# tprelle/janusgraph

Measured on AMD Instinct MI355X. Metric: GTEPS for PageRank iter + BFS, RMAT-24/26, 1/2/4/8 GPUs; % of HBM peak, higher is better.
Workload: dtype f64

## Files before the change

janusgraph_amd/csrc/jg_cc.hip:

```cpp
#include <climits>
#include <cstdio>
#include <cstdlib>

#include "jg_frontier.h"
#include "jg_pull.h"

namespace jg {

namespace {

constexpr int kCcMaxIterations = 100;

struct CcOp {
    using T = int32_t;
    const int32_t* __restrict__ msg;
    int32_t* __restrict__ msg_out;
    int32_t* __restrict__ label;
    int32_t* __restrict__ changed;
    VecPos pos;
    __device__ __forceinline__ int32_t identity() const { return INT_MAX; }
    __device__ __forceinline__ int32_t combine(int32_t a, int32_t b) const { return a < b ? a : b; }
    __device__ __forceinline__ int32_t gather(int32_t c) const { return msg[c]; }
    __device__ __forceinline__ const int32_t* vec() const { return msg; }
    __device__ __forceinline__ int32_t shfl_xor(int32_t v, int o) const { return __shfl_xor(v, o, kWave); }
    __device__ __forceinline__ int32_t shfl_up(int32_t v, int d) const { return __shfl_up(v, d, kWave); }
    __device__ __forceinline__ bool active(int64_t) const { return true; }
    __device__ __forceinline__ void finalize(int64_t row, int32_t m) const {
        if (m < label[row]) {
            label[row] = m;
            msg_out[pos(row)] = m;
            *changed = 1;
        } else {
            msg_out[pos(row)] = INT_MAX;
        }
    }
};

__device__ __forceinline__ int digits_of(uint64_t x) {
    int d = 1;
    while (d < 20 && x >= 10ull) { x /= 10ull; ++d; }
    return d;
}

__global__ void lex_digits_kernel(const int64_t* __restrict__ vid, int64_t n, uint64_t* __restrict__ keys,
                                  uint32_t* __restrict__ vals) {
    for (int64_t i = (int64_t)blockIdx.x * blockDim.x + threadIdx.x; i < n; i += (int64_t)gridDim.x * blockDim.x) {
        keys[i] = (uint64_t)digits_of((uint64_t)vid[i]);
        vals[i] = (uint32_t)i;
    }
}

__global__ void lex_padded_kernel(const int64_t* __restrict__ vid, const uint32_t* __restrict__ vals, int64_t n,
                                  uint64_t* __restrict__ keys) {
    for (int64_t i = (int64_t)blockIdx.x * blockDim.x + threadIdx.x; i < n; i += (int64_t)gridDim.x * blockDim.x) {
        uint64_t x = (uint64_t)vid[vals[i]];
        for (int d = digits_of(x); d < 19; ++d) x *= 10ull;
        keys[i] = x;
    }
}

__global__ void lex_rank_scatter_kernel(const uint32_t* __restrict__ vals, int64_t n, int32_t* __restrict__ rank_of) {
    for (int64_t r = (int64_t)blockIdx.x * blockDim.x + threadIdx.x; r < n; r += (int64_t)gridDim.x * blockDim.x)
        rank_of[vals[r]] = (int32_t)r;
}

__global__ void iota_i64_kernel(int64_t* __restrict__ p, int64_t n) {
    for (int64_t i = (int64_t)blockIdx.x * blockDim.x + threadIdx.x; i < n; i += (int64_t)gridDim.x * blockDim.x) p[i] = i;
}

__global__ void vid_of_rank_kernel(const uint32_t* __restrict__ vals, const int64_t* __restrict__ vid, int64_t n,
                                   int64_t* __restrict__ vor) {
    for (int64_t r = (int64_t)blockIdx.x * blockDim.x + threadIdx.x; r < n; r += (int64_t)gridDim.x * blockDim.x)
        vor[r] = vid[vals[r]];
}

__global__ void gather_i32_kernel(const int32_t* __restrict__ src, const int32_t* __restrict__ idx, int64_t n,
                                  int32_t* __restrict__ out) {
    for (int64_t i = (int64_t)blockIdx.x * blockDim.x + threadIdx.x; i < n; i += (int64_t)gridDim.x * blockDim.x)
// ... 1566 lines not shown
```

janusgraph_amd/csrc/jg_combine.hip:

```cpp
#include <climits>
#include <vector>

#include "jg_internal.h"
#include "jg_prim.h"
#include "jg_pull.h"

namespace jg {

namespace {

template <int OP>
struct Combine {
    __device__ static __forceinline__ int64_t identity() {
        return OP == JG_COMBINE_SUM ? 0 : OP == JG_COMBINE_MIN ? LLONG_MAX : LLONG_MIN;
    }
    __device__ static __forceinline__ int64_t apply(int64_t a, int64_t b) {
        if (OP == JG_COMBINE_SUM) return (int64_t)((uint64_t)a + (uint64_t)b);
        if (OP == JG_COMBINE_MIN) return b < a ? b : a;
        return b > a ? b : a;
    }
};

template <int OP>
__device__ __forceinline__ int64_t finish(int64_t acc, int wrap32) {
    return (OP == JG_COMBINE_SUM && wrap32) ? (int64_t)(int32_t)(uint32_t)acc : acc;
}

template <int OP>
struct CombOp {
    using T = long long;
    const long long* __restrict__ x;
    long long* __restrict__ x_out;
    VecPos pos;
    int wrap32;
    __device__ __forceinline__ long long identity() const { return Combine<OP>::identity(); }
    __device__ __forceinline__ long long combine(long long a, long long b) const { return Combine<OP>::apply(a, b); }
    __device__ __forceinline__ long long gather(int32_t c) const { return x[c]; }
    __device__ __forceinline__ const long long* vec() const { return x; }
    __device__ __forceinline__ long long shfl_xor(long long v, int o) const { return __shfl_xor(v, o, kWave); }
    __device__ __forceinline__ long long shfl_up(long long v, int d) const { return __shfl_up(v, d, kWave); }
    __device__ __forceinline__ bool active(int64_t) const { return true; }
    __device__ __forceinline__ void finalize(int64_t row, long long acc) const {
        x_out[pos(row)] = finish<OP>(acc, wrap32);
    }
};

__global__ void has_entries_kernel(const int64_t* __restrict__ row_ptr, int64_t rows, uint8_t* __restrict__ f) {
    for (int64_t r = (int64_t)blockIdx.x * blockDim.x + threadIdx.x; r < rows; r += (int64_t)gridDim.x * blockDim.x)
        f[r] = row_ptr[r + 1] > row_ptr[r];
}

template <int OP>
void launch_step(const Csr& c, const PullPlan& plan, long long* hub_partial, long long* split_partial,
                 const int64_t* x_in, int64_t* x_out, VecPos pos, int wrap32, hipStream_t s) {
    const CombOp<OP> op{reinterpret_cast<const long long*>(x_in), reinterpret_cast<long long*>(x_out), pos, wrap32};
    launch_pull(c, plan, op, hub_partial, s, nullptr, nullptr, split_partial);
}

}

void combine_run(Graph& g, int direction, int combiner, int wrap32, const int64_t* init, int steps, int64_t* out,
                 uint8_t* received_out) {
    if (direction < JG_DIR_OUT || direction > JG_DIR_BOTH) fail(JG_ERR_ARG, "direction must be JG_DIR_OUT/IN/BOTH");
    if (combiner < JG_COMBINE_SUM || combiner > JG_COMBINE_MAX) fail(JG_ERR_ARG, "unknown combiner");
    if (steps < 0) fail(JG_ERR_ARG, "negative step count");
    const uint32_t adj = direction == JG_DIR_OUT ? JG_ADJ_OUT : direction == JG_DIR_IN ? JG_ADJ_IN : JG_ADJ_BOTH;
    if (!(g.flags & adj))
        fail(JG_ERR_UNSUPPORTED, std::string("graph was built without the ") +
                                     (direction == JG_DIR_OUT ? "OUT" : direction == JG_DIR_IN ? "IN" : "BOTH") +
                                     " adjacency");
    const size_t ns = g.shards.size();
    struct St {
        DevBuf<int64_t> x[2];
        DevBuf<uint8_t> recv;
        DevBuf<long long> hub_partial, split_partial;
        int64_t len = 0;
        VecPos pos;
    };
    std::vector<St> st(ns);
    for (size_t i = 0; i < ns; ++i) {
        Shard& sh = *g.shards[i];
        DeviceGuard dg(sh);
        hipStream_t s = sh.stream;
        St& t = st[i];
        const Csr& c = adj == JG_ADJ_OUT ? sh.out : adj == JG_ADJ_IN ? sh.in : sh.both;
        if (adj == JG_ADJ_OUT) {
            t.len = g.padded_len();
            t.pos.base = (int64_t)sh.index * g.S;
            if (!sh.plan_out_built) {
                build_pull_plan(sh, sh.out, sh.plan_out, g.padded_len(), g.padded_len(), 8);
                sh.plan_out_built = true;
            }
        } else {
// ... 105 lines not shown
```

janusgraph_amd/csrc/jg_pagerank.hip:

```cpp
#include <cstdlib>

#include "jg_pull.h"
#include "jg_scatter.h"

namespace jg {

namespace {

struct PrOp {
    using T = double;
    const double* __restrict__ x;
    double* __restrict__ contrib_out;
    double* __restrict__ rank;
    const int32_t* __restrict__ outdeg;
    VecPos pos;
    double damping, teleport;
    bool write_rank;
    __device__ __forceinline__ double identity() const { return 0.0; }
    __device__ __forceinline__ double combine(double a, double b) const { return __dadd_rn(a, b); }
    __device__ __forceinline__ double gather(int32_t c) const { return x[c]; }
    __device__ __forceinline__ const double* vec() const { return x; }
    __device__ __forceinline__ double shfl_xor(double v, int o) const { return __shfl_xor(v, o, kWave); }
    __device__ __forceinline__ double shfl_up(double v, int d) const { return __shfl_up(v, d, kWave); }
    __device__ __forceinline__ bool active(int64_t) const { return true; }
    __device__ __forceinline__ void finalize(int64_t row, double s) const {
        const double r = __dadd_rn(__dmul_rn(damping, s), teleport);
        if (write_rank) rank[row] = r;
        contrib_out[pos(row)] = r / (double)outdeg[row];
    }
};

__global__ void pr_init_kernel(const int32_t* __restrict__ outdeg, int64_t rows, VecPos pos, double initial,
                               double* __restrict__ contrib, double* __restrict__ rank) {
    for (int64_t l = (int64_t)blockIdx.x * blockDim.x + threadIdx.x; l < rows; l += (int64_t)gridDim.x * blockDim.x) {
        rank[l] = initial;
        contrib[pos(l)] = initial / (double)outdeg[l];
    }
}

void exchange_contrib(Graph& g, int which) {
    std::vector<void*> bufs;
    for (auto& sp : g.shards) bufs.push_back(sp->pr_contrib[which].peer());
    exchange_vec(g, JG_ADJ_IN, bufs, sizeof(double), ncclFloat64);
}

}

void pagerank_begin(Graph& g, double damping, int64_t vertex_count) {
    if (!(g.flags & JG_ADJ_IN)) fail(JG_ERR_UNSUPPORTED, "PageRank needs a graph built with JG_ADJ_IN");
    if (vertex_count == 0) fail(JG_ERR_ARG, "vertexCount must be non-zero");
    for (auto& sp : g.shards) {
        Shard& sh = *sp;
        DeviceGuard dg(sh);
        const int64_t len = g.vec_len(sh, JG_ADJ_IN);
        for (int k = 0; k < 2; ++k) {
            if (sh.pr_contrib[k].size() != (size_t)len) sh.pr_contrib[k].alloc(len);
            JG_HIP(hipMemsetAsync(sh.pr_contrib[k].get(), 0, sh.pr_contrib[k].bytes(), sh.stream));
        }
        if (sh.pr_rank.size() != (size_t)std::max<int64_t>(sh.rows, 1)) {
            const char* f = std::getenv("JG_VDEV_FAULT");
            if (f && *f && *f != '0' && sh.index > 0) {
                DeviceGuard d0(*g.shards[0]);
                sh.pr_rank.alloc(std::max<int64_t>(sh.rows, 1));
            } else {
                sh.pr_rank.alloc(std::max<int64_t>(sh.rows, 1));
            }
        }
        if (sh.pr_hub_partial.size() != (size_t)std::max<int64_t>(sh.plan_in.num_chunks, 1))
            sh.pr_hub_partial.alloc(std::max<int64_t>(sh.plan_in.num_chunks, 1));
        if (sh.pr_split_partial.size() != (size_t)sh.plan_in.split_partial_len()) {
            sh.pr_split_partial.alloc(sh.plan_in.split_partial_len());
        }
        const double initial = 1.0 / (double)vertex_count;
        if (sh.rows > 0) {
            pr_init_kernel<<<grid_for(sh.rows), kBlock, 0, sh.stream>>>(sh.out_degree.get(), sh.rows,
                                                                        g.vec_pos(sh, JG_ADJ_IN), initial,
// ... 65 lines not shown
```

janusgraph_amd/csrc/jg_pull.h:

```cpp
#pragma once

#include "jg_internal.h"
#include "jg_prim.h"

namespace jg {

struct PullArgs {
    const int64_t* __restrict__ row_ptr;
    const int32_t* __restrict__ col;
    const int64_t* __restrict__ chunk_row;
    const int64_t* __restrict__ chunk_begin;
    const int64_t* __restrict__ chunk_end;
    const int64_t* __restrict__ hub_chunk_ptr;
    int64_t num_chunks;
    int64_t num_hub_rows;
    int64_t class_row_begin[kNumClasses];
    int64_t class_row_end[kNumClasses];
    int64_t class_block_begin[kNumClasses + 1];
    int64_t block_offset;
    int64_t skip_rows;
    int runs;
    int64_t run_begin[kRunMax + 1];
    int64_t run_ptr[kRunMax + 1];
};

inline PullArgs make_pull_args(const Csr& csr, const PullPlan& p, bool light = false) {
    PullArgs a;
    a.row_ptr = csr.row_ptr.get();
    a.col = csr.col.get();
    a.chunk_row = p.chunk_row.get();
    a.chunk_begin = p.chunk_begin.get();
    a.chunk_end = p.chunk_end.get();
    a.hub_chunk_ptr = p.hub_chunk_ptr.get();
    a.num_chunks = p.num_chunks;
    a.num_hub_rows = p.num_hub_rows;
    for (int c = 0; c < kNumClasses; ++c) {
        a.class_row_begin[c] = light ? p.light_row_begin[c] : p.class_row_begin[c];
        a.class_row_end[c] = light ? p.light_row_end[c] : p.class_row_end[c];
    }
    for (int c = 0; c <= kNumClasses; ++c) a.class_block_begin[c] = light ? p.light_block_begin[c] : p.class_block_begin[c];
    a.block_offset = 0;
    a.skip_rows = light ? p.split_rows : 0;
    a.runs = p.runs;
    for (int d = 0; d <= kRunMax; ++d) {
        a.run_begin[d] = p.run_begin[d];
        a.run_ptr[d] = p.run_ptr[d];
    }
    return a;
}

template <class Op>
struct GlobalGather {
    const Op& op;
// ... 146 lines not shown
            T t = red[0];
#pragma unroll
            for (int w = 1; w < kBlock / kWave; ++w) t = op.combine(t, red[w]);
            hub_partial[b] = t;
        }
        return;
    }
    pull_block_rows<Op, U>(a, op, GlobalGather<Op>{op}, b, (int)threadIdx.x);
}

template <class Op, int U>
__global__ __launch_bounds__(kBlock) void pull_kernel(PullArgs a, Op op, typename Op::T* __restrict__ hub_partial) {
    pull_block<Op, U>(a, op, hub_partial, (int64_t)blockIdx.x + a.block_offset);
}

template <class Op>
__global__ void pull_hub_finalize_kernel(PullArgs a, Op op, const typename Op::T* __restrict__ hub_partial) {
    using T = typename Op::T;
    for (int64_t h = (int64_t)blockIdx.x * blockDim.x + threadIdx.x; h < a.num_hub_rows;
         h += (int64_t)gridDim.x * blockDim.x) {
        const int64_t c0 = a.hub_chunk_ptr[h], c1 = a.hub_chunk_ptr[h + 1];
        if (a.chunk_row[c0] < a.skip_rows) continue;
        T acc = op.identity();
        for (int64_t k = c0; k < c1; ++k) acc = op.combine(acc, hub_partial[k]);
        op.finalize(a.chunk_row[c0], acc);
    }
}

constexpr int kMergeThreads = 1024;
constexpr int kMergeWaves = kMergeThreads / kWave;
constexpr int kMergeEpl = kMergeTask / kWave;
constexpr int kMergeLdsBytes = 160 * 1024;

struct MergeArgs {
    const uint4* __restrict__ pack_a;
    const uint32_t* __restrict__ pack_b;
    const uint8_t* __restrict__ heads;
    const int32_t* __restrict__ meta;
    const int64_t* __restrict__ sub_begin;
    const int64_t* __restrict__ sub_end;
    const int64_t* __restrict__ sub_base;
    int64_t tasks;
    int bits;
    int stage;
    const uint32_t* __restrict__ live;
};

struct HotSegs {
    int32_t hs = 0;
    int tbits = 31;
    int nseg = 1;
};

template <class Op>
struct SliceGather {
    using T = typename Op::T;
    const Op& op;
    lds_ptr<const T> lds;
    uint32_t hg;
    int sb;
    int bits;
    uint32_t hmask, h;
    uint32_t idcell;
    __device__ __forceinline__ bool is_hot(uint32_t loc) const { return ((loc >> 4) & ((1u << sb) - 1u)) < hg; }
    __device__ __forceinline__ T hot(uint32_t loc, bool valid) const {
        const uint32_t g = loc >> 4, j = g & ((1u << sb) - 1u), seg = g >> sb;
        return lds[valid && j < hg ? (((seg * hg + j) << 4) | (loc & 15u)) : idcell];
    }
    __device__ __forceinline__ int32_t col(uint32_t loc) const {
        const uint32_t x = (loc >> 4) << bits;
        const uint32_t hx = (x ^ (x >> 8) ^ (x >> 16) ^ (x >> 24)) & hmask;
        return (int32_t)(((x | (h ^ hx)) << 4) | (loc & 15u));
    }
    __device__ __forceinline__ T cold(uint32_t loc, bool valid, bool lds_on) const {
        T v = op.identity();
        if (valid && !(lds_on && is_hot(loc))) v = op.gather(col(loc));
        return v;
    }
};

template <int W>
__device__ __forceinline__ uint32_t unpack_entry(const uint32_t (&d)[W / 4], int u) {
    const int o = W * u, i = o >> 5, sh = o & 31;
    uint32_t v = d[i] >> sh;
    if (sh + W > 32) v |= d[i + 1] << (32 - sh);
    if constexpr (W < 32) v &= (1u << W) - 1u;
    return v;
}

template <class Op, bool LDS, int PW>
__global__ __launch_bounds__(kMergeThreads) void pull_merge_kernel(MergeArgs a, Op op, typename Op::T* __restrict__ partial,
                                                                   typename Op::T* __restrict__ carry, HotSegs hs,
                                                                   int temporal) {
    using T = typename Op::T;
    extern __shared__ __align__(16) unsigned char merge_lds[];
    const int S = 1 << a.bits;
    const int xs = S < kXcds ? S : kXcds;
    const int rep = kXcds / xs;
    const int per = S / xs;
    const int w = (int)(blockIdx.x >> 3), W = (int)(gridDim.x >> 3);
    const int xcd = (int)(blockIdx.x & (kXcds - 1));
    const int wave = threadIdx.x / kWave, lane = threadIdx.x % kWave;
    lds_ptr<T> hotv = (lds_ptr<T>)merge_lds;
    const int gshift = 4 + a.bits;
    const int hg = hs.hs >> gshift;
    const int nl = hs.nseg * hg;
    lds_ptr<T> stg = hotv + (nl * 16 + 1) + wave * a.stage;
    lds_ptr<uint32_t> tctr = (lds_ptr<uint32_t>)(hotv + (nl * 16 + 1) + kMergeWaves * a.stage);
    const int rounds = temporal ? per : 1;
    const uint32_t hmask = (1u << a.bits) - 1u;
    auto image_line = [&](int seg, int j, int hh) {
        const int64_t grp = ((int64_t)seg << (hs.tbits - gshift)) + j;
        return (grp << a.bits) + (int64_t)(hh ^ (sub_hash(grp << gshift) & hmask));
    };
    for (int rd = 0; rd < rounds; ++rd) {
    const int h = (xcd % xs) | ((temporal ? rd : w % per) << 3);
    const int64_t g = (int64_t)(temporal ? w : w / per) * rep + xcd / xs;
    const int64_t G = (int64_t)(temporal ? W : W / per) * rep;
    if constexpr (LDS) {
        if (rd > 0) __syncthreads();
        constexpr int kStage = 8;
        constexpr int kUnit = 16 / (int)sizeof(T);
        static_assert(16 % sizeof(T) == 0 && kUnit <= 16, "16-byte staging units");
        const unsigned char* src = reinterpret_cast<const unsigned char*>(op.vec());
        const int units = nl * 16 / kUnit;
        using u4 = uint32_t __attribute__((ext_vector_type(4)));
        lds_ptr<u4> hv4 = (lds_ptr<u4>)merge_lds;
        for (int q0 = 0; q0 < units; q0 += kStage * kMergeThreads) {
            u4 buf[kStage];
#pragma unroll
            for (int u = 0; u < kStage; ++u) {
                const int q = q0 + u * kMergeThreads + (int)threadIdx.x;
                const int i = q * kUnit, sg = i >> 4;
                int seg = 0, j = sg;
                if (hs.nseg > 1) {
                    seg = sg / hg;
                    j = sg - seg * hg;
                }
                buf[u] = u4{0, 0, 0, 0};
                if (q < units)
                    buf[u] = *reinterpret_cast<const u4*>(src + (image_line(seg, j, h) * 16 + (i & 15)) * (int64_t)sizeof(T));
            }
#pragma unroll
            for (int u = 0; u < kStage; ++u) {
                const int q = q0 + u * kMergeThreads + (int)threadIdx.x;
                if (q < units) hv4[q] = buf[u];
            }
        }
        if (threadIdx.x == 0) {
            hotv[nl * 16] = op.identity();
            *tctr = 0u;
        }
        __syncthreads();
    }
    const SliceGather<Op> lg{op,       hotv, (uint32_t)hg, hs.tbits - gshift, a.bits, (1u << a.bits) - 1u, (uint32_t)h,
                             (uint32_t)nl * 16u};
    const int64_t base = a.sub_base[h];
    const int64_t ntask = a.sub_base[h + 1] - base;
    const int64_t hbegin = a.sub_begin[h], hend = a.sub_end[h];
    constexpr bool dyn = LDS;
    const int64_t grot = (g + rd) % G;
    auto task_of = [&](int64_t j) { return j * G + grot; };
    auto grab = [&]() -> int64_t {
        uint32_t j = 0;
        if (lane == 0) j = __hip_atomic_fetch_add(tctr, 1u, __ATOMIC_RELAXED, __HIP_MEMORY_SCOPE_WORKGROUP);
        return task_of((int64_t)__builtin_amdgcn_readfirstlane(j));
    };
    int64_t jstat = wave;
    auto advance = [&]() -> int64_t {
        if (dyn) return grab();
        jstat += kMergeWaves;
        return task_of(jstat);
    };
    auto dead = [&](int64_t kk) -> bool {
        if (a.live == nullptr || kk >= ntask) return false;
        const uint64_t tt = (uint64_t)(base + kk);
        const uint32_t wd = __builtin_amdgcn_readfirstlane(a.live[tt >> 5]);
        return ((wd >> (tt & 31)) & 1u) == 0;
    };
    int64_t k = dyn ? grab() : task_of(jstat);
    while (dead(k)) k = advance();
    if (k >= ntask) continue;
    static_assert(kMergeEpl == 8, "a lane chunk is 8 entries");
    constexpr int DB = PW / 4 - 4;
    auto chunk = [&](int64_t kk) { return (hbegin >> 3) + kk * kWave + lane; };
    auto meta_idx = [&](int64_t kk) { return 2 * (base + kk) + (lane & 1); };
    auto head_idx = [&](int64_t kk) { return (base + kk) * kWave + lane; };
    auto ld = [](const auto* p) { return *p; };
    using v4u = uint32_t __attribute__((ext_vector_type(4)));
    using v2u = uint32_t __attribute__((ext_vector_type(2)));
    auto load_chunk = [&](int64_t kk, uint32_t (&d)[PW / 4]) {
        const int64_t x = chunk(kk);
        const v4u va = ld(reinterpret_cast<const v4u*>(a.pack_a) + x);
        d[0] = va.x, d[1] = va.y, d[2] = va.z, d[3] = va.w;
        if constexpr (DB == 1) {
            d[4] = ld(a.pack_b + x);
        } else if constexpr (DB == 2) {
            const v2u vb = ld(reinterpret_cast<const v2u*>(a.pack_b) + x);
            d[4] = vb.x, d[5] = vb.y;
        } else {
            const v4u vb = ld(reinterpret_cast<const v4u*>(a.pack_b) + x);
            d[4] = vb.x, d[5] = vb.y, d[6] = vb.z, d[7] = vb.w;
        }
    };
    uint32_t cd[PW / 4];
    load_chunk(k, cd);
    uint32_t hb = ld(a.heads + head_idx(k));
    int32_t mw = ld(a.meta + meta_idx(k));
    for (;;) {
        const int64_t t = base + k;
        const int64_t e0 = hbegin + k * kMergeTask;
        const int n = (int)min((int64_t)kMergeTask, hend - e0);
        uint32_t loc[kMergeEpl];
#pragma unroll
        for (int u = 0; u < kMergeEpl; ++u) loc[u] = unpack_entry<PW>(cd, u);
        const int32_t j0 = __builtin_amdgcn_readlane(mw, 0);
        const bool carry_in = __builtin_amdgcn_readlane(mw, 1) != 0;
        const uint32_t hbc = hb;
        T v[kMergeEpl];
        if constexpr (LDS) {
            T vg[kMergeEpl], vl[kMergeEpl];
#pragma unroll
            for (int u = 0; u < kMergeEpl; ++u) vl[u] = lg.hot(loc[u], kMergeEpl * lane + u < n);
#pragma unroll
            for (int u = 0; u < kMergeEpl; ++u) vg[u] = lg.cold(loc[u], kMergeEpl * lane + u < n, true);
#pragma unroll
            for (int u = 0; u < kMergeEpl; ++u) v[u] = op.combine(vl[u], vg[u]);
        } else {
#pragma unroll
            for (int u = 0; u < kMergeEpl; ++u) v[u] = lg.cold(loc[u], kMergeEpl * lane + u < n, false);
        }
        int64_t kn = advance();
        while (dead(kn)) kn = advance();
        if (kn < ntask) {
            load_chunk(kn, cd);
            hb = ld(a.heads + head_idx(kn));
            mw = ld(a.meta + meta_idx(kn));
        }
        const int cnt = __builtin_popcount(hbc);
        int incl = cnt;
#pragma unroll
        for (int d = 1; d < kWave; d <<= 1) {
            const int o = __shfl_up(incl, d, kWave);
            if (lane >= d) incl += o;
        }
        const int hbase = incl - cnt;
        const bool valid_lane = kMergeEpl * lane < n;
        const int H = __builtin_amdgcn_readlane(incl, kWave - 1);
        const bool staged = LDS && H <= a.stage;
        auto store_partial = [&](int64_t j, T val) { partial[j] = val; };
        auto emit = [&](int hh, T val) {
            if (staged) {
                stg[hh] = val;
                return;
            }
            if (hh == 0 && carry_in) carry[t] = val;
            else store_partial(j0 + hh, val);
        };
        const int fh = hbc ? __builtin_ctz(hbc) : kMergeEpl;
        T pre = op.identity(), run = op.identity();
        int run_h = hbase - 1;
#pragma unroll
        for (int u = 0; u < kMergeEpl; ++u) {
            if (u < fh) {
                pre = u == 0 ? v[u] : op.combine(pre, v[u]);
            } else if ((hbc >> u) & 1u) {
                if (u > fh) emit(run_h, run);
                run = v[u];
                ++run_h;
            } else {
                run = op.combine(run, v[u]);
            }
        }
        T x = fh < kMergeEpl ? run : pre;
        int f = fh < kMergeEpl ? 1 : 0;
        int xh = run_h;
#pragma unroll
        for (int d = 1; d < kWave; d <<= 1) {
            const T xu = op.shfl_up(x, d);
            const int fu = __shfl_up(f, d, kWave);
            const int hu = __shfl_up(xh, d, kWave);
            if (lane >= d) {
                if (!f) {
                    x = op.combine(xu, x);
                    xh = hu;
                }
                f |= fu;
            }
        }
        const T in_x = op.shfl_up(x, 1);
        const int in_h = __shfl_up(xh, 1, kWave);
        if (valid_lane) {
            if (lane > 0 && fh < kMergeEpl) emit(in_h, fh > 0 ? op.combine(in_x, pre) : in_x);
            if (kMergeEpl * (lane + 1) >= n) {
                if (fh < kMergeEpl) emit(run_h, run);
                else emit(in_h, lane > 0 ? op.combine(in_x, pre) : pre);
            }
        }
        if (staged) {
            __builtin_amdgcn_fence(__ATOMIC_RELEASE, "wavefront");
            __builtin_amdgcn_wave_barrier();
            __builtin_amdgcn_fence(__ATOMIC_ACQUIRE, "wavefront");
            for (int i = lane; i < H; i += kWave) {
                const T val = stg[i];
                if (i == 0 && carry_in) carry[t] = val;
                else store_partial(j0 + i, val);
            }
            __builtin_amdgcn_fence(__ATOMIC_RELEASE, "wavefront");
            __builtin_amdgcn_wave_barrier();
            __builtin_amdgcn_fence(__ATOMIC_ACQUIRE, "wavefront");
        }
        if (kn >= ntask) break;
        k = kn;
    }
    }
}

constexpr int kMaxBands = 4;
struct FixupBands {
    const int32_t* meta[kMaxBands];
    int64_t task_begin[kMaxBands + 1];
    int64_t part_off[kMaxBands], carry_off[kMaxBands];
    int n;
};
template <class Op>
__global__ void pull_merge_fixup_kernel(FixupBands fb, Op op, typename Op::T* __restrict__ split_partial) {
    using T = typename Op::T;
    for (int64_t x = (int64_t)blockIdx.x * blockDim.x + threadIdx.x; x < fb.task_begin[fb.n];
         x += (int64_t)gridDim.x * blockDim.x) {
        int b = 0;
        while (x >= fb.task_begin[b + 1]) ++b;
        const int64_t t = x - fb.task_begin[b], tasks = fb.task_begin[b + 1] - fb.task_begin[b];
        const int32_t* __restrict__ meta = fb.meta[b];
        T* __restrict__ partial = split_partial + fb.part_off[b];
        const T* __restrict__ carry = split_partial + fb.carry_off[b];
        const int64_t tp = t > 0 ? t - 1 : 0, tn = t + 1 < tasks ? t + 1 : t;
        const int32_t f = meta[2 * t + 1], j = meta[2 * t];
        const int32_t pf = meta[2 * tp + 1], pj = meta[2 * tp];
        const int32_t nf = meta[2 * tn + 1], nj = meta[2 * tn];
        const T c = carry[t], cn = carry[tn];
        if (!f || (t > 0 && pf && pj == j)) continue;
        T acc = op.combine(partial[j], c);
        if (tn != t && nf && nj == j) {
            acc = op.combine(acc, cn);
            for (int64_t u = t + 2; u < tasks && meta[2 * u + 1] && meta[2 * u] == j; ++u) acc = op.combine(acc, carry[u]);
        }
        partial[j] = acc;
    }
}

struct FinalizeBands {
    const uint2* sub_word[kMaxBands];
    int64_t row_begin[kMaxBands];
    int64_t row_end[kMaxBands];
    int64_t part_off[kMaxBands];
    int bits[kMaxBands];
    int n;
};
template <class Op>
__device__ __forceinline__ void slice_finalize_row(int64_t r, const Op& op, const FinalizeBands& fb,
                                                   const typename Op::T* __restrict__ partial) {
    using T = typename Op::T;
    int b = 0;
// ... 13 lines not shown
            wd[u] = h0 + u < S ? sw[(int64_t)(h0 + u) * W + wi] : make_uint2(0u, 0u);
    };
    load_words(0, wc);
    for (int h0 = 0; h0 < S; h0 += 8) {
        int32_t j[8];
        T v[8];
#pragma unroll
        for (int u = 0; u < 8; ++u) j[u] = (wc[u].x & me) ? (int32_t)wc[u].y + __popc(wc[u].x & below) : -1;
        if (h0 + 8 < S) load_words(h0 + 8, wn);
#pragma unroll
        for (int u = 0; u < 8; ++u) v[u] = j[u] >= 0 ? part[j[u]] : op.identity();
#pragma unroll
        for (int u = 0; u < 8; ++u)
            if (j[u] >= 0) {
                acc = first ? v[u] : op.combine(acc, v[u]);
                first = false;
            }
#pragma unroll
        for (int u = 0; u < 8; ++u) wc[u] = wn[u];
    }
    op.finalize(r, acc);
}

template <class Op>
__global__ void pull_slice_finalize_kernel(int64_t row0, int64_t rows, Op op, FinalizeBands fb,
                                           const typename Op::T* __restrict__ partial) {
    for (int64_t r = row0 + (int64_t)blockIdx.x * blockDim.x + threadIdx.x; r < rows; r += (int64_t)gridDim.x * blockDim.x)
        slice_finalize_row(r, op, fb, partial);
}

template <class Op, int U>
__global__ __launch_bounds__(kBlock) void pull_light_finalize_kernel(PullArgs a, Op op,
                                                                     typename Op::T* __restrict__ hub_partial,
                                                                     FinalizeBands fb,
                                                                     const typename Op::T* __restrict__ partial,
                                                                     int64_t split_rows, int64_t fin_blocks,
                                                                     int64_t fin_row0) {
    const int64_t b = blockIdx.x;
    if (b < fin_blocks) {
        const int64_t r = fin_row0 + b * kBlock + threadIdx.x;
        if (r < split_rows) slice_finalize_row<Op>(r, op, fb, partial);
        return;
    }
    pull_block<Op, U>(a, op, hub_partial, b - fin_blocks + a.block_offset);
}


template <class Op>
void launch_pull(const Csr& csr, const PullPlan& plan, const Op& op, typename Op::T* hub_partial, hipStream_t s,
                 Ctx* prof_ctx = nullptr, Shard* prof_shard = nullptr, typename Op::T* split_partial = nullptr,
                 bool skip_empty = false, const uint32_t* const* task_live = nullptr, int64_t caller_rows = 0) {
    using T = typename Op::T;
    const bool split = tune().pull_split && plan.split_rows > 0 && split_partial != nullptr;
    size_t band0 = 0;
    if (caller_rows > 0) {
        while (band0 < plan.bands.size() && plan.bands[band0]->row_end <= caller_rows) ++band0;
        if (!split || band0 == 0 || plan.bands[band0 - 1]->row_end != caller_rows)
            fail(JG_ERR_UNSUPPORTED, "launch_pull: caller rows must end a prefix of the split bands");
    }
    PullArgs a = make_pull_args(csr, plan, split);
    if (skip_empty) a.class_block_begin[kNumClasses] = a.class_block_begin[kZeroClass];
    const int64_t blocks = a.class_block_begin[kNumClasses];
    if (prof_ctx) prof_record_start(*prof_ctx, *prof_shard);
    if (split) {
        static bool attr = false;
        if (!attr) {
            JG_HIP(hipFuncSetAttribute((const void*)pull_merge_kernel<Op, true, 20>,
                                       hipFuncAttributeMaxDynamicSharedMemorySize, kMergeLdsBytes));
            JG_HIP(hipFuncSetAttribute((const void*)pull_merge_kernel<Op, true, 24>,
                                       hipFuncAttributeMaxDynamicSharedMemorySize, kMergeLdsBytes));
            JG_HIP(hipFuncSetAttribute((const void*)pull_merge_kernel<Op, true, 32>,
                                       hipFuncAttributeMaxDynamicSharedMemorySize, kMergeLdsBytes));
            attr = true;
        }
        for (size_t bi = band0; bi < plan.bands.size(); ++bi) {
            const SliceBand& bd = *plan.bands[bi];
            if (bd.tasks == 0) continue;
            int stage = tune().merge_stage[std::min<size_t>(bi, 3)];
            if (stage < 0) {
                const double heads = (double)bd.subrows / (double)std::max<int64_t>(bd.tasks, 1);
                stage = 128;
                while (stage < 4.0 * heads && stage < 256) stage *= 2;
            }
            MergeArgs ma{bd.pack_a.get(), bd.pack_b.get(), bd.heads.get(), bd.meta.get(), bd.sub_begin.get(),
                         bd.sub_end.get(), bd.sub_base.get(), bd.tasks, bd.bits, stage,
                         task_live ? task_live[bi] : nullptr};
            T* part = split_partial + bd.part_off;
            T* carry = split_partial + bd.carry_off;
            const int64_t S = 1ll << bd.bits, gsz = 16 * S;
            const unsigned grid = (unsigned)std::max<int64_t>(S, (int64_t)device_cu_count() / S * S);
            const int64_t stage_bytes = (int64_t)kMergeWaves * stage * (int64_t)sizeof(T);
            const int64_t hot_max = (int64_t)((kMergeLdsBytes - stage_bytes - 16) / (int64_t)sizeof(T) - 16) * S;
            HotSegs hs;
            hs.tbits = plan.seg_tbits;
            hs.nseg = plan.nseg;
            const int64_t seg_cap = plan.nseg == 1 ? plan.col_space : (1ll << plan.seg_tbits) - gsz;
            hs.hs = plan.lds_ok ? (int32_t)(std::min<int64_t>(hot_max / plan.nseg, seg_cap) / gsz * gsz) : 0;
            const int temporal = tune().merge_temporal == 2 || (tune().merge_temporal == 1 && plan.temporal);
            const size_t lds = hs.hs > 0 ? (size_t)(hs.nseg * (hs.hs / S) + 1) * sizeof(T) + (size_t)stage_bytes + 16 : 0;
            auto go = [&](auto kern) { kern<<<grid, kMergeThreads, lds, s>>>(ma, op, part, carry, hs, temporal); };
            if (hs.hs > 0) {
                if (bd.width == 20) go(pull_merge_kernel<Op, true, 20>);
                else if (bd.width == 24) go(pull_merge_kernel<Op, true, 24>);
                else go(pull_merge_kernel<Op, true, 32>);
            } else {
                if (bd.width == 20) go(pull_merge_kernel<Op, false, 20>);
                else if (bd.width == 24) go(pull_merge_kernel<Op, false, 24>);
                else go(pull_merge_kernel<Op, false, 32>);
            }
            JG_LAUNCH_CHECK();
        }
        FixupBands fx{};
        for (size_t bi = band0; bi < plan.bands.size(); ++bi) {
            const auto& bp = plan.bands[bi];
            if (fx.n == kMaxBands) fail(JG_ERR_UNSUPPORTED, "too many split bands");
            fx.meta[fx.n] = bp->meta.get();
            fx.part_off[fx.n] = bp->part_off;
            fx.carry_off[fx.n] = bp->carry_off;
            fx.task_begin[fx.n + 1] = fx.task_begin[fx.n] + bp->tasks;
            ++fx.n;
        }
        if (fx.task_begin[fx.n] > 0) {
            pull_merge_fixup_kernel<Op><<<grid_for(fx.task_begin[fx.n], kBlock, 0), kBlock, 0, s>>>(fx, op, split_partial);
            JG_LAUNCH_CHECK();
        }
    }
    auto launch = [&](unsigned grid) {
        pull_kernel<Op, 4><<<grid, kBlock, 0, s>>>(a, op, hub_partial);
        JG_LAUNCH_CHECK();
    };
    FinalizeBands fb{};
    if (split) {
        for (const auto& bp : plan.bands) {
            if (fb.n == kMaxBands) fail(JG_ERR_UNSUPPORTED, "too many split bands");
            fb.sub_word[fb.n] = bp->sub_word.get();
            fb.row_begin[fb.n] = bp->row_begin;
            fb.row_end[fb.n] = bp->row_end;
            fb.part_off[fb.n] = bp->part_off;
            fb.bits[fb.n] = bp->bits;
            ++fb.n;
        }
    }
    const bool fuse = split && !pull_split_launches();
    if (fuse) {
        const int64_t fin_blocks = (plan.split_rows - caller_rows + kBlock - 1) / kBlock;
        const unsigned grid = (unsigned)(fin_blocks + blocks);
        pull_light_finalize_kernel<Op, 4><<<grid, kBlock, 0, s>>>(a, op, hub_partial, fb, split_partial, plan.split_rows,
                                                                  fin_blocks, caller_rows);
        JG_LAUNCH_CHECK();
    } else if (pull_split_launches()) {
        for (int c = 0; c < kNumClasses; ++c) {
            const int64_t b0 = a.class_block_begin[c], b1 = a.class_block_begin[c + 1];
            if (b1 <= b0) continue;
            a.block_offset = b0;
// ... 20 lines not shown
```

janusgraph_amd/csrc/jg_traverse.hip:

```cpp
#include <climits>
#include <initializer_list>
#include <type_traits>

#include <cstdio>

#include "jg_frontier.h"
#include "jg_pull.h"
#include "jg_scatter.h"

namespace jg {

namespace {

constexpr int kTdEdgesPerThread = 4;
constexpr int kBuBatch = 4;
constexpr int kBfsRing = 4;

__device__ __forceinline__ void wave_append(bool take, int32_t v, int32_t* __restrict__ queue,
                                            unsigned long long* __restrict__ size) {
    const uint64_t mask = __ballot(take);
    if (mask == 0) return;
    const int leader = __ffsll((unsigned long long)mask) - 1;
    unsigned long long base = 0;
    if (lane_id() == leader) base = atomicAdd(size, (unsigned long long)__popcll(mask));
// ... 309 lines not shown
                const int4 x = *reinterpret_cast<const int4*>(r.rank + v0);
                lab[0] = x.x, lab[1] = x.y, lab[2] = x.z, lab[3] = x.w;
            } else {
#pragma unroll
                for (int k = 0; k < kQ; ++k) lab[k] = v0 + k < rows ? r.rank[v0 + k] : 0;
            }
            if (in) {
                const int4 x = *reinterpret_cast<const int4*>(r.parent + v0);
                par[0] = x.x, par[1] = x.y, par[2] = x.z, par[3] = x.w;
            } else {
#pragma unroll
                for (int k = 0; k < kQ; ++k) par[k] = v0 + k < r.ne ? r.parent[v0 + k] : 0;
            }
#pragma unroll
            for (int k = 0; k < kQ; ++k) {
                const int64_t v = v0 + k;
                bool least = true;
                dep[k] = -1;
                if (v < r.ne) {
                    const int32_t m = r.minr[par[k]];
                    least = lab[k] == m;
                    if (least) {
                        deg[k] = deg_rp[v + 1] - deg_rp[v];
                        take[k] = deg[k] > 0;
                    }
                    lab[k] = m;
                    dep[k] = take[k] ? 0 : -1;
                }
                sn[k] = least;
            }
            if (full) {
                *reinterpret_cast<int4*>(r.parent + v0) = make_int4(lab[0], lab[1], lab[2], lab[3]);
                *reinterpret_cast<uint32_t*>(seen + v0) =
                    (uint32_t)sn[0] | (uint32_t)sn[1] << 8 | (uint32_t)sn[2] << 16 | (uint32_t)sn[3] << 24;
            } else {
                for (int k = 0; k < kQ && v0 + k < rows; ++k) {
                    r.parent[v0 + k] = lab[k];
                    seen[v0 + k] = sn[k];
                }
            }
            if (in) *reinterpret_cast<int4*>(depth + v0) = make_int4(dep[0], dep[1], dep[2], dep[3]);
            else
                for (int k = 0; k < kQ && v0 + k < r.ne; ++k) depth[v0 + k] = dep[k];
        }
#pragma unroll
        for (int k = 0; k < kQ; ++k) app.append(take[k], (int32_t)(v0 + k), deg[k], queue, qoff, packed);
    }
    app.final(queue, qoff, packed);
}

constexpr int kMsLevelWords = 12;
struct MsBfsOp {
    using T = unsigned long long;
    const T* __restrict__ F;
    T* __restrict__ Fout;
    T* __restrict__ visited;
    int32_t* __restrict__ depth;
    uint8_t* __restrict__ depth8;
    unsigned long long* __restrict__ nwl;
    int32_t* __restrict__ changed;
    int64_t rows;
    VecPos pos;
    int32_t lvl;
    const T* live;
    __device__ __forceinline__ T identity() const { return 0ull; }
    __device__ __forceinline__ T combine(T a, T b) const { return a | b; }
    __device__ __forceinline__ T gather(int32_t c) const { return F[c]; }
    __device__ __forceinline__ const T* vec() const { return F; }
    __device__ __forceinline__ T shfl_xor(T v, int o) const { return __shfl_xor(v, o, kWave); }
    __device__ __forceinline__ T shfl_up(T v, int d) const { return __shfl_up(v, d, kWave); }
    __device__ __forceinline__ bool active(int64_t row) const { return (~visited[row] & *live) != 0ull; }
    __device__ __forceinline__ void finalize(int64_t row, T acc) const {
        T nw = acc & ~visited[row] & *live;
        Fout[pos(row)] = nw;
        if (nwl) nwl[row] = nw;
        if (nw) {
            visited[row] |= nw;
            if (changed) *changed = 1;
            while (nw) {
                const int s = __ffsll(nw) - 1;
                if (depth8) depth8[(int64_t)s * rows + row] = (uint8_t)lvl;
                else if (depth) depth[(int64_t)s * rows + row] = lvl;
                nw &= nw - 1;
            }
        }
    }
};

__global__ __launch_bounds__(kRedThreads) void msbfs_live_kernel(const unsigned long long* __restrict__ F, int64_t len,
                                                                 unsigned long long* __restrict__ live) {
    __shared__ unsigned long long red[kRedWaves];
    unsigned long long m = 0;
    for (int64_t i = (int64_t)blockIdx.x * blockDim.x + threadIdx.x; i < len; i += (int64_t)gridDim.x * blockDim.x)
        m |= F[i];
    m = block_reduce(m, OrU64{}, red);
    if (threadIdx.x == 0 && m) atomicOr(live, m);
}

__global__ __launch_bounds__(kRedThreads) void msbfs_scan_kernel(const unsigned long long* __restrict__ F, int64_t rows,
                                                                 const int64_t* __restrict__ push_rp,
                                                                 unsigned long long* __restrict__ live,
                                                                 unsigned long long* __restrict__ packed) {
    __shared__ unsigned long long red_or[kRedWaves], red_n[kRedWaves];
    unsigned long long m = 0, cnt = 0;
    for (int64_t v = (int64_t)blockIdx.x * blockDim.x + threadIdx.x; v < rows; v += (int64_t)gridDim.x * blockDim.x) {
        const unsigned long long w = F[v];
        if (w) {
            m |= w;
            cnt += (1ull << kPackShift) + (unsigned long long)(push_rp[v + 1] - push_rp[v]);
        }
    }
    m = block_reduce(m, OrU64{}, red_or);
    cnt = block_reduce(cnt, AddU64{}, red_n);
    if (threadIdx.x == 0) {
        if (m) atomicOr(live, m);
        if (cnt) atomicAdd(packed, cnt);
    }
}

__global__ __launch_bounds__(kBlock) void msbfs_todo_kernel(const unsigned long long* __restrict__ visited,
                                                            int64_t row0, int64_t nrows,
                                                            const unsigned long long* __restrict__ live,
                                                            unsigned long long* __restrict__ todo) {
// ... 3392 lines not shown
```

Before: 364.8.

## Streamline merge-kernel segmented scan and add single-segment hot-LDS specialization

```diff
diff --git a/janusgraph_amd/csrc/jg_cc.hip b/janusgraph_amd/csrc/jg_cc.hip
--- a/janusgraph_amd/csrc/jg_cc.hip
+++ b/janusgraph_amd/csrc/jg_cc.hip
@@ -23,7 +23,6 @@
     __device__ __forceinline__ int32_t gather(int32_t c) const { return msg[c]; }
     __device__ __forceinline__ const int32_t* vec() const { return msg; }
     __device__ __forceinline__ int32_t shfl_xor(int32_t v, int o) const { return __shfl_xor(v, o, kWave); }
-    __device__ __forceinline__ int32_t shfl_up(int32_t v, int d) const { return __shfl_up(v, d, kWave); }
     __device__ __forceinline__ bool active(int64_t) const { return true; }
     __device__ __forceinline__ void finalize(int64_t row, int32_t m) const {
         if (m < label[row]) {
diff --git a/janusgraph_amd/csrc/jg_combine.hip b/janusgraph_amd/csrc/jg_combine.hip
--- a/janusgraph_amd/csrc/jg_combine.hip
+++ b/janusgraph_amd/csrc/jg_combine.hip
@@ -38,7 +38,6 @@
     __device__ __forceinline__ long long gather(int32_t c) const { return x[c]; }
     __device__ __forceinline__ const long long* vec() const { return x; }
     __device__ __forceinline__ long long shfl_xor(long long v, int o) const { return __shfl_xor(v, o, kWave); }
-    __device__ __forceinline__ long long shfl_up(long long v, int d) const { return __shfl_up(v, d, kWave); }
     __device__ __forceinline__ bool active(int64_t) const { return true; }
     __device__ __forceinline__ void finalize(int64_t row, long long acc) const {
         x_out[pos(row)] = finish<OP>(acc, wrap32);
diff --git a/janusgraph_amd/csrc/jg_pagerank.hip b/janusgraph_amd/csrc/jg_pagerank.hip
--- a/janusgraph_amd/csrc/jg_pagerank.hip
+++ b/janusgraph_amd/csrc/jg_pagerank.hip
@@ -21,7 +21,6 @@
     __device__ __forceinline__ double gather(int32_t c) const { return x[c]; }
     __device__ __forceinline__ const double* vec() const { return x; }
     __device__ __forceinline__ double shfl_xor(double v, int o) const { return __shfl_xor(v, o, kWave); }
-    __device__ __forceinline__ double shfl_up(double v, int d) const { return __shfl_up(v, d, kWave); }
     __device__ __forceinline__ bool active(int64_t) const { return true; }
     __device__ __forceinline__ void finalize(int64_t row, double s) const {
         const double r = __dadd_rn(__dmul_rn(damping, s), teleport);
diff --git a/janusgraph_amd/csrc/jg_pull.h b/janusgraph_amd/csrc/jg_pull.h
--- a/janusgraph_amd/csrc/jg_pull.h
+++ b/janusgraph_amd/csrc/jg_pull.h
@@ -1,4 +1,6 @@
 #pragma once
+
+#include <type_traits>
 
 #include "jg_internal.h"
 #include "jg_prim.h"
@@ -251,7 +253,7 @@
     int nseg = 1;
 };
 
-template <class Op>
+template <class Op, bool MSEG = true>
 struct SliceGather {
     using T = typename Op::T;
     const Op& op;
@@ -261,8 +263,12 @@
     int bits;
     uint32_t hmask, h;
     uint32_t idcell;
-    __device__ __forceinline__ bool is_hot(uint32_t loc) const { return ((loc >> 4) & ((1u << sb) - 1u)) < hg; }
+    __device__ __forceinline__ bool is_hot(uint32_t loc) const {
+        if constexpr (!MSEG) return loc < (hg << 4);
+        return ((loc >> 4) & ((1u << sb) - 1u)) < hg;
+    }
     __device__ __forceinline__ T hot(uint32_t loc, bool valid) const {
+        if constexpr (!MSEG) return lds[valid && loc < (hg << 4) ? loc : idcell];
         const uint32_t g = loc >> 4, j = g & ((1u << sb) - 1u), seg = g >> sb;
         return lds[valid && j < hg ? (((seg * hg + j) << 4) | (loc & 15u)) : idcell];
     }
@@ -287,7 +293,24 @@
     return v;
 }
 
-template <class Op, bool LDS, int PW>
+template <class T>
+__device__ __forceinline__ T lane_up(T v, int lane, int d) {
+    static_assert(sizeof(T) % 4 == 0, "whole dwords");
+    int w[sizeof(T) / 4];
+    __builtin_memcpy(w, &v, sizeof(T));
+    const int addr = ((lane - d) & (kWave - 1)) << 2;
+#pragma unroll
+    for (size_t i = 0; i < sizeof(T) / 4; ++i) w[i] = __builtin_amdgcn_ds_bpermute(addr, w[i]);
+    __builtin_memcpy(&v, w, sizeof(T));
+    return v;
+}
+
+template <class Op, class = void>
+struct op_task_live : std::false_type {};
+template <class Op>
+struct op_task_live<Op, std::void_t<decltype(Op::kTaskLive)>> : std::bool_constant<Op::kTaskLive> {};
+
+template <class Op, bool LDS, int PW, bool MSEG = false>
 __global__ __launch_bounds__(kMergeThreads) void pull_merge_kernel(MergeArgs a, Op op, typename Op::T* __restrict__ partial,
                                                                    typename Op::T* __restrict__ carry, HotSegs hs,
                                                                    int temporal) {
@@ -304,8 +327,8 @@
     const int gshift = 4 + a.bits;
     const int hg = hs.hs >> gshift;
     const int nl = hs.nseg * hg;
-    lds_ptr<T> stg = hotv + (nl * 16 + 1) + wave * a.stage;
-    lds_ptr<uint32_t> tctr = (lds_ptr<uint32_t>)(hotv + (nl * 16 + 1) + kMergeWaves * a.stage);
+    lds_ptr<T> stg = hotv + (nl * 16 + 1) + wave * (a.stage + 1);
+    lds_ptr<uint32_t> tctr = (lds_ptr<uint32_t>)(hotv + (nl * 16 + 1) + kMergeWaves * (a.stage + 1));
     const int rounds = temporal ? per : 1;
     const uint32_t hmask = (1u << a.bits) - 1u;
     auto image_line = [&](int seg, int j, int hh) {
@@ -352,7 +375,7 @@
         }
         __syncthreads();
     }
-    const SliceGather<Op> lg{op,       hotv, (uint32_t)hg, hs.tbits - gshift, a.bits, (1u << a.bits) - 1u, (uint32_t)h,
+    const SliceGather<Op, MSEG> lg{op,       hotv, (uint32_t)hg, hs.tbits - gshift, a.bits, (1u << a.bits) - 1u, (uint32_t)h,
                              (uint32_t)nl * 16u};
     const int64_t base = a.sub_base[h];
     const int64_t ntask = a.sub_base[h + 1] - base;
@@ -372,6 +395,7 @@
         return task_of(jstat);
     };
     auto dead = [&](int64_t kk) -> bool {
+        if constexpr (!op_task_live<Op>::value) return false;
         if (a.live == nullptr || kk >= ntask) return false;
         const uint64_t tt = (uint64_t)(base + kk);
         const uint32_t wd = __builtin_amdgcn_readfirstlane(a.live[tt >> 5]);
@@ -436,67 +460,83 @@
             hb = ld(a.heads + head_idx(kn));
             mw = ld(a.meta + meta_idx(kn));
         }
-        const int cnt = __builtin_popcount(hbc);
-        int incl = cnt;
-#pragma unroll
-        for (int d = 1; d < kWave; d <<= 1) {
-            const int o = __shfl_up(incl, d, kWave);
-            if (lane >= d) incl += o;
-        }
-        const int hbase = incl - cnt;
+        static_assert(kMergeEpl < 16, "a lane's head count has 4 bits");
+        const uint32_t cnt = (uint32_t)__builtin_popcount(hbc);
+        int hbase = 0;
+        int H = 0;
+#pragma unroll
+        for (int b = 0; b < 4; ++b) {
+            const uint64_t cb = __ballot((cnt >> b) & 1u);
+            hbase += (int)__builtin_amdgcn_mbcnt_hi((uint32_t)(cb >> 32), __builtin_amdgcn_mbcnt_lo((uint32_t)cb, 0u)) << b;
+            H += __builtin_popcountll(cb) << b;
+        }
         const bool valid_lane = kMergeEpl * lane < n;
-        const int H = __builtin_amdgcn_readlane(incl, kWave - 1);
         const bool staged = LDS && H <= a.stage;
+        const uint64_t hm = __ballot(hbc != 0u);
+        const uint64_t hml = hm << (kWave - 1 - lane);
+        const int gap = hml ? __builtin_clzll(hml) : kWave;
+        const int reach = min(lane, gap);
+        const int in_h = hbase - 1;
         auto store_partial = [&](int64_t j, T val) { partial[j] = val; };
-        auto emit = [&](int hh, T val) {
-            if (staged) {
-                stg[hh] = val;
-                return;
-            }
-            if (hh == 0 && carry_in) carry[t] = val;
-            else store_partial(j0 + hh, val);
+        auto scan_in = [&](T x) -> T {
+#pragma unroll
+            for (int d = 1; d < kWave; d <<= 1) {
+                const T xu = lane_up(x, lane, d);
+                if (reach >= d) x = op.combine(xu, x);
+            }
+            return lane_up(x, lane, 1);
         };
-        const int fh = hbc ? __builtin_ctz(hbc) : kMergeEpl;
-        T pre = op.identity(), run = op.identity();
-        int run_h = hbase - 1;
-#pragma unroll
-        for (int u = 0; u < kMergeEpl; ++u) {
-            if (u < fh) {
-                pre = u == 0 ? v[u] : op.combine(pre, v[u]);
-            } else if ((hbc >> u) & 1u) {
-                if (u > fh) emit(run_h, run);
-                run = v[u];
-                ++run_h;
-            } else {
-                run = op.combine(run, v[u]);
-            }
-        }
-        T x = fh < kMergeEpl ? run : pre;
-        int f = fh < kMergeEpl ? 1 : 0;
-        int xh = run_h;
-#pragma unroll
-        for (int d = 1; d < kWave; d <<= 1) {
-            const T xu = op.shfl_up(x, d);
-            const int fu = __shfl_up(f, d, kWave);
-            const int hu = __shfl_up(xh, d, kWave);
-            if (lane >= d) {
-                if (!f) {
-                    x = op.combine(xu, x);
-                    xh = hu;
+        auto fold_direct = [&]() {
+            auto emit = [&](int hh, T val) {
+                if (hh == 0 && carry_in) carry[t] = val;
+                else store_partial(j0 + hh, val);
+            };
+            const int fh = hbc ? __builtin_ctz(hbc) : kMergeEpl;
+            T pre = op.identity(), run = op.identity();
+            int run_h = hbase - 1;
+#pragma unroll
+            for (int u = 0; u < kMergeEpl; ++u) {
+                if (u < fh) {
+                    pre = u == 0 ? v[u] : op.combine(pre, v[u]);
+                } else if ((hbc >> u) & 1u) {
+                    if (u > fh) emit(run_h, run);
+                    run = v[u];
+                    ++run_h;
+                } else {
+                    run = op.combine(run, v[u]);
                 }
-                f |= fu;
-            }
-        }
-        const T in_x = op.shfl_up(x, 1);
-        const int in_h = __shfl_up(xh, 1, kWave);
-        if (valid_lane) {
-            if (lane > 0 && fh < kMergeEpl) emit(in_h, fh > 0 ? op.combine(in_x, pre) : in_x);
-            if (kMergeEpl * (lane + 1) >= n) {
-                if (fh < kMergeEpl) emit(run_h, run);
-                else emit(in_h, lane > 0 ? op.combine(in_x, pre) : pre);
-            }
-        }
-        if (staged) {
+            }
+            const T in_x = scan_in(fh < kMergeEpl ? run : pre);
+            if (valid_lane) {
+                if (lane > 0 && fh < kMergeEpl) emit(in_h, fh > 0 ? op.combine(in_x, pre) : in_x);
+                if (kMergeEpl * (lane + 1) >= n) {
+                    if (fh < kMergeEpl) emit(run_h, run);
+                    else emit(in_h, lane > 0 ? op.combine(in_x, pre) : pre);
+                }
+            }
+        };
+        auto fold_staged = [&]() {
+            const int dump = a.stage;
+            bool seen = (hbc & 1u) != 0u;
+            int slot = in_h + (int)(hbc & 1u);
+            T acc = v[0], pre = op.identity();
+#pragma unroll
+            for (int u = 1; u < kMergeEpl; ++u) {
+                const bool head = ((hbc >> u) & 1u) != 0u;
+                stg[head && seen ? slot : dump] = acc;
+                pre = head && !seen ? acc : pre;
+                const T sum = op.combine(acc, v[u]);
+                acc = head ? v[u] : sum;
+                slot += head ? 1 : 0;
+                seen = seen || head;
+            }
+            pre = seen ? pre : acc;
+            const T in_x = scan_in(acc);
+            const T joined = op.combine(in_x, pre);
+            stg[valid_lane && lane > 0 && seen ? in_h : dump] = (hbc & 1u) ? in_x : joined;
+            const bool last = valid_lane && kMergeEpl * (lane + 1) >= n;
+            const T whole = lane > 0 ? joined : pre;
+            stg[last ? (seen ? slot : in_h) : dump] = seen ? acc : whole;
             __builtin_amdgcn_fence(__ATOMIC_RELEASE, "wavefront");
             __builtin_amdgcn_wave_barrier();
             __builtin_amdgcn_fence(__ATOMIC_ACQUIRE, "wavefront");
@@ -508,6 +548,12 @@
             __builtin_amdgcn_fence(__ATOMIC_RELEASE, "wavefront");
             __builtin_amdgcn_wave_barrier();
             __builtin_amdgcn_fence(__ATOMIC_ACQUIRE, "wavefront");
+        };
+        if constexpr (LDS) {
+            if (staged) fold_staged();
+            else fold_direct();
+        } else {
+            fold_direct();
         }
         if (kn >= ntask) break;
         k = kn;
@@ -627,6 +673,8 @@
                  bool skip_empty = false, const uint32_t* const* task_live = nullptr, int64_t caller_rows = 0) {
     using T = typename Op::T;
     const bool split = tune().pull_split && plan.split_rows > 0 && split_partial != nullptr;
+    if (task_live != nullptr && !op_task_live<Op>::value)
+        fail(JG_ERR_UNSUPPORTED, "launch_pull: this Op does not declare kTaskLive");
     size_t band0 = 0;
     if (caller_rows > 0) {
         while (band0 < plan.bands.size() && plan.bands[band0]->row_end <= caller_rows) ++band0;
@@ -646,6 +694,12 @@
                                        hipFuncAttributeMaxDynamicSharedMemorySize, kMergeLdsBytes));
             JG_HIP(hipFuncSetAttribute((const void*)pull_merge_kernel<Op, true, 32>,
                                        hipFuncAttributeMaxDynamicSharedMemorySize, kMergeLdsBytes));
+            JG_HIP(hipFuncSetAttribute((const void*)pull_merge_kernel<Op, true, 20, true>,
+                                       hipFuncAttributeMaxDynamicSharedMemorySize, kMergeLdsBytes));
+            JG_HIP(hipFuncSetAttribute((const void*)pull_merge_kernel<Op, true, 24, true>,
+                                       hipFuncAttributeMaxDynamicSharedMemorySize, kMergeLdsBytes));
+            JG_HIP(hipFuncSetAttribute((const void*)pull_merge_kernel<Op, true, 32, true>,
+                                       hipFuncAttributeMaxDynamicSharedMemorySize, kMergeLdsBytes));
             attr = true;
         }
         for (size_t bi = band0; bi < plan.bands.size(); ++bi) {
@@ -664,7 +718,7 @@
             T* carry = split_partial + bd.carry_off;
             const int64_t S = 1ll << bd.bits, gsz = 16 * S;
             const unsigned grid = (unsigned)std::max<int64_t>(S, (int64_t)device_cu_count() / S * S);
-            const int64_t stage_bytes = (int64_t)kMergeWaves * stage * (int64_t)sizeof(T);
+            const int64_t stage_bytes = (int64_t)kMergeWaves * (stage + 1) * (int64_t)sizeof(T);
             const int64_t hot_max = (int64_t)((kMergeLdsBytes - stage_bytes - 16) / (int64_t)sizeof(T) - 16) * S;
             HotSegs hs;
             hs.tbits = plan.seg_tbits;
@@ -674,7 +728,11 @@
             const int temporal = tune().merge_temporal == 2 || (tune().merge_temporal == 1 && plan.temporal);
             const size_t lds = hs.hs > 0 ? (size_t)(hs.nseg * (hs.hs / S) + 1) * sizeof(T) + (size_t)stage_bytes + 16 : 0;
             auto go = [&](auto kern) { kern<<<grid, kMergeThreads, lds, s>>>(ma, op, part, carry, hs, temporal); };
-            if (hs.hs > 0) {
+            if (hs.hs > 0 && hs.nseg > 1) {
+                if (bd.width == 20) go(pull_merge_kernel<Op, true, 20, true>);
+                else if (bd.width == 24) go(pull_merge_kernel<Op, true, 24, true>);
+                else go(pull_merge_kernel<Op, true, 32, true>);
+            } else if (hs.hs > 0) {
                 if (bd.width == 20) go(pull_merge_kernel<Op, true, 20>);
                 else if (bd.width == 24) go(pull_merge_kernel<Op, true, 24>);
                 else go(pull_merge_kernel<Op, true, 32>);
diff --git a/janusgraph_amd/csrc/jg_traverse.hip b/janusgraph_amd/csrc/jg_traverse.hip
--- a/janusgraph_amd/csrc/jg_traverse.hip
+++ b/janusgraph_amd/csrc/jg_traverse.hip
@@ -385,6 +385,7 @@
 constexpr int kMsLevelWords = 12;
 struct MsBfsOp {
     using T = unsigned long long;
+    static constexpr bool kTaskLive = true;
     const T* __restrict__ F;
     T* __restrict__ Fout;
     T* __restrict__ visited;
@@ -401,7 +402,6 @@
     __device__ __forceinline__ T gather(int32_t c) const { return F[c]; }
     __device__ __forceinline__ const T* vec() const { return F; }
     __device__ __forceinline__ T shfl_xor(T v, int o) const { return __shfl_xor(v, o, kWave); }
-    __device__ __forceinline__ T shfl_up(T v, int d) const { return __shfl_up(v, d, kWave); }
     __device__ __forceinline__ bool active(int64_t row) const { return (~visited[row] & *live) != 0ull; }
     __device__ __forceinline__ void finalize(int64_t row, T acc) const {
         T nw = acc & ~visited[row] & *live;
```

After: 382.1 (median of 6 runs). 1.05x the previous value.
